# samxuxiang/BrepGen

Measured on NVIDIA H100. Metric: B-reps/sec (1000-step ABC cascade), higher is better.
Workload: dtype f16 x f16 -> f32 (wgmma; split hi+lo weights on in/out-proj; fp32 residual/LN/softmax)

## Files before the change

### brepgen_b200/csrc/attn.cu

```cuda
#include <math.h>

#include "bg_internal.h"
#include "ptx.cuh"


namespace bg {

namespace {

constexpr int DH = 64;
constexpr int NHEAD = 12;
constexpr int DMODEL = 768;
constexpr int BQ = 128;
constexpr int TILE_BYTES = 128 * DH * 2;
constexpr int ST = 2;
constexpr int OFF_Q = 0;
constexpr int OFF_K = TILE_BYTES;
constexpr int OFF_V = OFF_K + ST * TILE_BYTES;
constexpr int OFF_BAR = OFF_V + ST * TILE_BYTES;
constexpr int OFF_MASKW = OFF_BAR + 256;
constexpr int MAX_KB = ATTN_MAX_L / 128;
constexpr int SMEM_BYTES = OFF_MASKW + MAX_KB * 16 + 1024;
constexpr int THREADS = 384;
constexpr int CONSUMER_THREADS = 256;

struct AttnParams {
  __half* out;
  int ldo;
  int B, L, nkb;
  const uint8_t* key_mask;
  const int* blk_list;
  const int* blk_count;
  const uint32_t* blk_words;
  const int* seq_row0;
  const int* seq_len;
  float scale_log2;
};

__device__ __forceinline__ float quad_max(float v) {
  v = fmaxf(v, __shfl_xor_sync(0xffffffffu, v, 1));
  return fmaxf(v, __shfl_xor_sync(0xffffffffu, v, 2));
}
__device__ __forceinline__ float quad_sum(float v) {
  v += __shfl_xor_sync(0xffffffffu, v, 1);
  return v + __shfl_xor_sync(0xffffffffu, v, 2);
}

struct Ring {
  int stage = 0;
  uint32_t phase = 0;
  __device__ __forceinline__ void advance() {
    if (++stage == ST) {
      stage = 0;
      phase ^= 1u;
    }
  }
};

__device__ __forceinline__ void issue_qk(float (&sc)[64], uint32_t q_addr, uint32_t k_addr) {
#pragma unroll
  for (int k = 0; k < DH / 16; ++k)
    wgmma_m64n128k16_ss(sc, make_sw128_desc(q_addr + k * 32), make_sw128_desc(k_addr + k * 32), k > 0 ? 1u : 0u);
  wgmma_commit();
}

__device__ __forceinline__ void issue_pv(float (&o)[DH / 2], const uint32_t (&pa)[8][4], uint32_t v_addr) {
#pragma unroll
  for (int kk = 0; kk < 8; ++kk) wgmma_m64n64k16_rs_bt(o, pa[kk], make_sw128_desc(v_addr + kk * 2048), 1u);
  wgmma_commit();
}

__device__ __forceinline__ void softmax_block(float (&sc)[64], const uint32_t* iw4, float (&m_run)[2], float (&l_run)[2],
                                              float (&alpha)[2], float c, int lane) {
  const uint4 iw = *reinterpret_cast<const uint4*>(iw4);
  if ((iw.x | iw.y | iw.z | iw.w) != 0) {
    const uint32_t inval[4] = {iw.x, iw.y, iw.z, iw.w};
#pragma unroll
    for (int i = 0; i < 16; ++i)
#pragma unroll
      for (int j = 0; j < 2; ++j) {
        const int key = 8 * i + 2 * (lane & 3) + j;
        if ((inval[key >> 5] >> (key & 31)) & 1u) {
          sc[4 * i + j] = -INFINITY;
          sc[4 * i + 2 + j] = -INFINITY;
        }
      }
  }
  float ref[2];
#pragma unroll
  for (int hr = 0; hr < 2; ++hr) {
    float mx = -INFINITY;
#pragma unroll
    for (int i = 0; i < 16; ++i) mx = fmaxf(mx, fmaxf(sc[4 * i + 2 * hr], sc[4 * i + 2 * hr + 1]));
    const float m_new = fmaxf(m_run[hr], quad_max(mx));
    ref[hr] = m_new == -INFINITY ? 0.f : m_new;
    alpha[hr] = ex2((m_run[hr] - ref[hr]) * c);
    m_run[hr] = m_new;
    l_run[hr] *= alpha[hr];
  }
  const float nm0 = -ref[0] * c, nm1 = -ref[1] * c;
#pragma unroll
  for (int i = 0; i < 16; ++i) {
    const float p0 = ex2(fmaf(sc[4 * i], c, nm0)), p1 = ex2(fmaf(sc[4 * i + 1], c, nm0));
    const float p2 = ex2(fmaf(sc[4 * i + 2], c, nm1)), p3 = ex2(fmaf(sc[4 * i + 3], c, nm1));
    l_run[0] += p0 + p1;
    l_run[1] += p2 + p3;
    sc[4 * i] = p0;
    sc[4 * i + 1] = p1;
    sc[4 * i + 2] = p2;
    sc[4 * i + 3] = p3;
  }
}

__device__ __forceinline__ void scale_o(float (&o)[DH / 2], const float (&alpha)[2]) {
#pragma unroll
  for (int i = 0; i < DH / 8; ++i) {
    o[4 * i] *= alpha[0];
    o[4 * i + 1] *= alpha[0];
    o[4 * i + 2] *= alpha[1];
    o[4 * i + 3] *= alpha[1];
  }
}

__device__ __forceinline__ void pack_p(uint32_t (&pa)[8][4], const float (&sc)[64]) {
#pragma unroll
  for (int i = 0; i < 16; ++i) {
    pa[i >> 1][(i & 1) * 2] = pack_half2(sc[4 * i], sc[4 * i + 1]);
    pa[i >> 1][(i & 1) * 2 + 1] = pack_half2(sc[4 * i + 2], sc[4 * i + 3]);
  }
}

__global__ void __launch_bounds__(THREADS, 1)
attn_kernel(const __grid_constant__ CUtensorMap tmQKV, const AttnParams p) {
  extern __shared__ uint8_t smem_raw[];
  uint8_t* smem = reinterpret_cast<uint8_t*>((reinterpret_cast<uintptr_t>(smem_raw) + 1023) & ~uintptr_t(1023));
  uint64_t* bars = reinterpret_cast<uint64_t*>(smem + OFF_BAR);
  uint64_t* q_full = bars;
  uint64_t* k_full = q_full + 1;
  uint64_t* k_empty = k_full + ST;
  uint64_t* v_full = k_empty + ST;
  uint64_t* v_empty = v_full + ST;

  const int warp = threadIdx.x >> 5;
  const int lane = threadIdx.x & 31;
  const int wg = threadIdx.x >> 7;
  const int qgrp = blockIdx.x, h = blockIdx.y, b = blockIdx.z;
  const int row0 = p.seq_row0 ? p.seq_row0[b] : b * p.L;
  const int len = p.seq_len ? p.seq_len[b] : p.L;
  if (qgrp * BQ >= len) return;
  const int nblk = p.blk_count ? p.blk_count[b] : (len + 127) / 128;
  const int* blist = p.blk_list ? p.blk_list + (size_t)b * p.nkb : nullptr;

  if (threadIdx.x == 0) {
    tma_prefetch_desc(&tmQKV);
    mbar_init(q_full, 1);
    for (int i = 0; i < ST; ++i) {
      mbar_init(&k_full[i], 1);
      mbar_init(&k_empty[i], CONSUMER_THREADS);
      mbar_init(&v_full[i], 1);
      mbar_init(&v_empty[i], CONSUMER_THREADS);
    }
    fence_barrier_init();
  }
  uint32_t* maskw = reinterpret_cast<uint32_t*>(smem + OFF_MASKW);
  if (p.blk_words || !p.key_mask) {
    for (int wi = threadIdx.x; wi < nblk * 4; wi += THREADS) {
      uint32_t w;
      if (p.blk_words) {
        w = p.blk_words[((size_t)b * p.nkb + (wi >> 2)) * 4 + (wi & 3)];
      } else {
        const int base = (wi >> 2) * 128 + (wi & 3) * 32;
        w = base + 32 <= len ? 0u : (base >= len ? 0xffffffffu : (0xffffffffu << (len - base)));
      }
      maskw[wi] = w;
    }
  } else {
    for (int wi = warp; wi < nblk * 4; wi += THREADS / 32) {
      const int kb = blist ? blist[wi >> 2] : (wi >> 2);
      const int key = kb * 128 + (wi & 3) * 32 + lane;
      bool bad = key >= len;
      if (!bad) bad = p.key_mask[(size_t)b * p.L + key] != 0;
      const uint32_t w = __ballot_sync(0xffffffffu, bad);
      if (lane == 0) maskw[wi] = w;
    }
  }
  __syncthreads();

  if (wg == 0) {
    setmaxnreg_dec<24>();
    if (warp == 0 && elect_one()) {
      mbar_arrive_expect_tx(q_full, TILE_BYTES);
      tma_load_2d(smem + OFF_Q, &tmQKV, q_full, h * DH, row0 + qgrp * BQ);
      Ring r;
      for (int it = 0; it < nblk; ++it, r.advance()) {
        const int kb = blist ? blist[it] : it;
        const int s = r.stage;
        mbar_wait(&k_empty[s], r.phase ^ 1u);
        mbar_arrive_expect_tx(&k_full[s], TILE_BYTES);
        tma_load_2d(smem + OFF_K + s * TILE_BYTES, &tmQKV, &k_full[s], DMODEL + h * DH, row0 + kb * 128);
        mbar_wait(&v_empty[s], r.phase ^ 1u);
        mbar_arrive_expect_tx(&v_full[s], TILE_BYTES);
        tma_load_2d(smem + OFF_V + s * TILE_BYTES, &tmQKV, &v_full[s], 2 * DMODEL + h * DH, row0 + kb * 128);
      }
    }
    return;
  }

  setmaxnreg_inc<240>();
  const int half = wg - 1;
  const int wq = warp & 3;
  const float c = p.scale_log2;
  const uint32_t q_addr = smem_u32(smem + OFF_Q) + half * 64 * 128;
  float m_run[2] = {-INFINITY, -INFINITY}, l_run[2] = {0.f, 0.f};
  float o[DH / 2];
#pragma unroll
  for (int i = 0; i < DH / 2; ++i) o[i] = 0.f;

  mbar_wait(q_full, 0);
  if (nblk > 0) {
    const uint32_t k_base = smem_u32(smem + OFF_K), v_base = smem_u32(smem + OFF_V);
    Ring kr, vr;
    float sc[64], alpha[2];
    uint32_t pa[8][4];

    mbar_wait(&k_full[kr.stage], kr.phase);
    wgmma_fence();
    issue_qk(sc, q_addr, k_base + kr.stage * TILE_BYTES);
    wgmma_wait<0>();
    wgmma_fence_operand(sc);
    mbar_arrive(&k_empty[kr.stage]);
    kr.advance();
    softmax_block(sc, maskw, m_run, l_run, alpha, c, lane);

#pragma unroll 1
    for (int it = 1; it < nblk; ++it) {
      wgmma_wait<0>();
      wgmma_fence_operand(o);
      if (it >= 2) {
        mbar_arrive(&v_empty[vr.stage]);
        vr.advance();
      }
      scale_o(o, alpha);
      pack_p(pa, sc);
      mbar_wait(&k_full[kr.stage], kr.phase);
      mbar_wait(&v_full[vr.stage], vr.phase);
      wgmma_fence_operand(o);
      wgmma_fence();
      issue_qk(sc, q_addr, k_base + kr.stage * TILE_BYTES);
      issue_pv(o, pa, v_base + vr.stage * TILE_BYTES);
      wgmma_wait<1>();
      wgmma_fence_operand(sc);
      mbar_arrive(&k_empty[kr.stage]);
      kr.advance();
      softmax_block(sc, maskw + it * 4, m_run, l_run, alpha, c, lane);
    }

    wgmma_wait<0>();
    wgmma_fence_operand(o);
    if (nblk >= 2) {
      mbar_arrive(&v_empty[vr.stage]);
      vr.advance();
    }
    scale_o(o, alpha);
    pack_p(pa, sc);
    mbar_wait(&v_full[vr.stage], vr.phase);
    wgmma_fence_operand(o);
    wgmma_fence();
    issue_pv(o, pa, v_base + vr.stage * TILE_BYTES);
    wgmma_wait<0>();
    wgmma_fence_operand(o);
    mbar_arrive(&v_empty[vr.stage]);
  }

#pragma unroll
  for (int hr = 0; hr < 2; ++hr) {
    const float l = quad_sum(l_run[hr]);
    const float inv = l > 0.f ? 1.f / l : 0.f;
    const int row = qgrp * BQ + half * 64 + wq * 16 + hr * 8 + (lane >> 2);
    if (row >= len) continue;
    __half* dst = p.out + ((size_t)row0 + row) * p.ldo + h * DH + 2 * (lane & 3);
#pragma unroll
    for (int i = 0; i < DH / 8; ++i)
      *reinterpret_cast<uint32_t*>(dst + 8 * i) = pack_half2(o[4 * i + 2 * hr] * inv, o[4 * i + 2 * hr + 1] * inv);
  }
}

__global__ void block_list_kernel(const uint8_t* __restrict__ key_mask, int L, int nkb, int* __restrict__ blk_list,
                                  int* __restrict__ blk_count, uint32_t* __restrict__ blk_words) {
  extern __shared__ int sm_bl[];
  int* pos = sm_bl;
  uint32_t* wds = reinterpret_cast<uint32_t*>(sm_bl + nkb);
  const int b = blockIdx.x;
  const int warp = threadIdx.x >> 5, lane = threadIdx.x & 31, nwarp = blockDim.x >> 5;
  for (int kb = warp; kb < nkb; kb += nwarp) {
    bool any = false;
#pragma unroll
    for (int c = 0; c < 4; ++c) {
      const int key = kb * 128 + c * 32 + lane;
      const bool bad = key >= L || key_mask[(size_t)b * L + key] != 0;
      const uint32_t w = __ballot_sync(0xffffffffu, bad);
      any = any || w != 0xffffffffu;
      if (lane == 0) wds[kb * 4 + c] = w;
    }
    if (lane == 0) pos[kb] = any ? 0 : -1;
  }
  __syncthreads();
  if (threadIdx.x == 0) {
    int n = 0;
    for (int kb = 0; kb < nkb; ++kb)
      if (pos[kb] == 0) {
        blk_list[(size_t)b * nkb + n] = kb;
        pos[kb] = n++;
      }
    blk_count[b] = n;
  }
  __syncthreads();
  if (blk_words)
    for (int i = threadIdx.x; i < nkb * 4; i += blockDim.x)
      if (pos[i >> 2] >= 0) blk_words[((size_t)b * nkb + pos[i >> 2]) * 4 + (i & 3)] = wds[i];
}

}

int launch_attention(cudaStream_t st, const AttnArgs& a) {
  BG_REQUIRE(a.qkv && a.out && a.B > 0 && a.L > 0, "attention: bad arguments");
  BG_REQUIRE(a.ldo % 8 == 0, "attention: output pitch must be a multiple of 8");
  BG_REQUIRE(a.L <= ATTN_MAX_L, "attention: sequence longer than 8192 tokens is not supported");
  BG_REQUIRE((a.blk_list == nullptr) == (a.blk_count == nullptr), "attention: blk_list and blk_count go together");
  CUtensorMap tm;
  BG_REQUIRE((a.seq_row0 == nullptr) == (a.seq_len == nullptr), "attention: seq_row0 and seq_len go together");
  BG_REQUIRE(a.seq_len == nullptr || (a.key_mask == nullptr && a.blk_list == nullptr), "attention: variable-length mode takes no mask");
  BG_TRY(make_tmap_2d_f16(&tm, a.qkv, (uint64_t)a.B * (uint64_t)a.L, 3 * DMODEL, 3 * DMODEL, 128));
  AttnParams p;
  p.out = a.out; p.ldo = a.ldo; p.B = a.B; p.L = a.L; p.nkb = (a.L + 127) / 128;
  p.key_mask = a.key_mask; p.blk_list = a.blk_list; p.blk_count = a.blk_count; p.blk_words = a.blk_words;
  p.seq_row0 = a.seq_row0; p.seq_len = a.seq_len;
  p.scale_log2 = 1.4426950408889634f / 8.0f;
  BG_TRY(ensure_dynamic_smem(reinterpret_cast<const void*>(&attn_kernel), SMEM_BYTES));
  dim3 grid((a.L + BQ - 1) / BQ, NHEAD, a.B);
  attn_kernel<<<grid, THREADS, SMEM_BYTES, st>>>(tm, p);
  return check_launch("attn_kernel launch");
}

int launch_build_block_list(cudaStream_t st, const uint8_t* key_mask, int B, int L, int* blk_list, int* blk_count,
                            uint32_t* blk_words) {
  BG_REQUIRE(key_mask && blk_list && blk_count && B > 0 && L > 0, "block list: bad arguments");
  const int nkb = (L + 127) / 128;
  block_list_kernel<<<B, 128, nkb * 5 * sizeof(int), st>>>(key_mask, L, nkb, blk_list, blk_count, blk_words);
  return check_launch("block_list_kernel launch");
}

}
```

### brepgen_b200/csrc/ptx.cuh

```cuda
#pragma once
#include <cuda.h>
#include <cuda_fp16.h>
#include <cuda_runtime.h>
#include <stdint.h>

namespace bg {

__device__ __forceinline__ uint32_t smem_u32(const void* p) { return (uint32_t)__cvta_generic_to_shared(p); }

__device__ __forceinline__ bool elect_one() {
  uint32_t pred;
  asm volatile(
      "{\n\t.reg .pred P;\n\t.reg .b32 R;\n\t"
      "elect.sync R|P, 0xffffffff;\n\t"
      "selp.b32 %0, 1, 0, P;\n\t}\n"
      : "=r"(pred));
  return pred != 0;
}

__device__ __forceinline__ void mbar_init(uint64_t* bar, uint32_t count) {
  asm volatile("mbarrier.init.shared::cta.b64 [%0], %1;" ::"r"(smem_u32(bar)), "r"(count));
}
__device__ __forceinline__ void fence_barrier_init() { asm volatile("fence.mbarrier_init.release.cluster;" ::: "memory"); }
__device__ __forceinline__ void mbar_arrive(uint64_t* bar) {
  asm volatile("mbarrier.arrive.shared::cta.b64 _, [%0];" ::"r"(smem_u32(bar)) : "memory");
}
__device__ __forceinline__ void mbar_arrive_expect_tx(uint64_t* bar, uint32_t bytes) {
  asm volatile("mbarrier.arrive.expect_tx.shared::cta.b64 _, [%0], %1;" ::"r"(smem_u32(bar)), "r"(bytes) : "memory");
}
__device__ __forceinline__ bool mbar_try_wait(uint64_t* bar, uint32_t parity) {
  uint32_t ok;
  asm volatile(
      "{\n\t.reg .pred P;\n\t"
      "mbarrier.try_wait.parity.shared::cta.b64 P, [%1], %2;\n\t"
      "selp.b32 %0, 1, 0, P;\n\t}\n"
      : "=r"(ok)
      : "r"(smem_u32(bar)), "r"(parity)
      : "memory");
  return ok != 0;
}
__device__ __forceinline__ void mbar_wait(uint64_t* bar, uint32_t parity) {
  uint32_t spins = 0;
  while (!mbar_try_wait(bar, parity)) {
    if (++spins > (1u << 26)) asm volatile("trap;");
  }
}

__device__ __forceinline__ void tma_prefetch_desc(const CUtensorMap* m) {
  asm volatile("prefetch.tensormap [%0];" ::"l"(reinterpret_cast<uint64_t>(m)) : "memory");
}
__device__ __forceinline__ void tma_load_2d(void* smem_dst, const CUtensorMap* m, uint64_t* bar, int c0, int c1) {
  asm volatile(
      "cp.async.bulk.tensor.2d.shared::cluster.global.mbarrier::complete_tx::bytes [%0], [%1, {%3, %4}], [%2];"
      ::"r"(smem_u32(smem_dst)), "l"(reinterpret_cast<uint64_t>(m)), "r"(smem_u32(bar)), "r"(c0), "r"(c1)
      : "memory");
}

__device__ __forceinline__ void tma_load_4d(void* smem_dst, const CUtensorMap* m, uint64_t* bar, int c0, int c1, int c2, int c3) {
  asm volatile(
      "cp.async.bulk.tensor.4d.shared::cluster.global.mbarrier::complete_tx::bytes [%0], [%1, {%3, %4, %5, %6}], [%2];"
      ::"r"(smem_u32(smem_dst)), "l"(reinterpret_cast<uint64_t>(m)), "r"(smem_u32(bar)), "r"(c0), "r"(c1), "r"(c2), "r"(c3)
      : "memory");
}

__device__ __forceinline__ void prefetch_l2_bulk(const void* p, uint32_t bytes) {
  asm volatile("cp.async.bulk.prefetch.L2.global [%0], %1;" ::"l"(reinterpret_cast<uint64_t>(p)), "r"(bytes) : "memory");
}

template <uint32_t N>
__device__ __forceinline__ void setmaxnreg_dec() { asm volatile("setmaxnreg.dec.sync.aligned.u32 %0;" ::"n"(N)); }
template <uint32_t N>
__device__ __forceinline__ void setmaxnreg_inc() { asm volatile("setmaxnreg.inc.sync.aligned.u32 %0;" ::"n"(N)); }

__device__ __forceinline__ uint64_t make_sw128_desc(uint32_t smem_addr, uint32_t sbo_bytes = 1024) {
  uint64_t d = 0;
  d |= (uint64_t)((smem_addr & 0x3FFFF) >> 4);
  d |= (uint64_t)1 << 16;
  d |= (uint64_t)((sbo_bytes >> 4) & 0x3FFF) << 32;
  d |= (uint64_t)1 << 62;
  return d;
}

__device__ __forceinline__ void wgmma_fence() { asm volatile("wgmma.fence.sync.aligned;" ::: "memory"); }
__device__ __forceinline__ void wgmma_commit() { asm volatile("wgmma.commit_group.sync.aligned;" ::: "memory"); }
template <int N>
__device__ __forceinline__ void wgmma_wait() { asm volatile("wgmma.wait_group.sync.aligned %0;" ::"n"(N) : "memory"); }
template <int R>
__device__ __forceinline__ void wgmma_fence_operand(float (&d)[R]) {
#pragma unroll
  for (int i = 0; i < R; ++i) asm volatile("" : "+f"(d[i])::"memory");
}

__device__ __forceinline__ void wgmma_m64n256k16_ss(float (&d)[128], uint64_t a_desc, uint64_t b_desc, uint32_t accumulate) {
  asm volatile(
      "{\n\t.reg .pred p;\n\t"
      "setp.ne.b32 p, %130, 0;\n\t"
      "wgmma.mma_async.sync.aligned.m64n256k16.f32.f16.f16 "
      "{%0, %1, %2, %3, %4, %5, %6, %7, %8, %9, %10, %11, %12, %13, %14, %15, "
      "%16, %17, %18, %19, %20, %21, %22, %23, %24, %25, %26, %27, %28, %29, %30, %31, "
      "%32, %33, %34, %35, %36, %37, %38, %39, %40, %41, %42, %43, %44, %45, %46, %47, "
      "%48, %49, %50, %51, %52, %53, %54, %55, %56, %57, %58, %59, %60, %61, %62, %63, "
      "%64, %65, %66, %67, %68, %69, %70, %71, %72, %73, %74, %75, %76, %77, %78, %79, "
      "%80, %81, %82, %83, %84, %85, %86, %87, %88, %89, %90, %91, %92, %93, %94, %95, "
      "%96, %97, %98, %99, %100, %101, %102, %103, %104, %105, %106, %107, %108, %109, %110, %111, "
      "%112, %113, %114, %115, %116, %117, %118, %119, %120, %121, %122, %123, %124, %125, %126, %127}, "
      "%128, %129, p, 1, 1, 0, 0;\n\t}\n"
      : "+f"(d[0]), "+f"(d[1]), "+f"(d[2]), "+f"(d[3]), "+f"(d[4]), "+f"(d[5]), "+f"(d[6]), "+f"(d[7]),
        "+f"(d[8]), "+f"(d[9]), "+f"(d[10]), "+f"(d[11]), "+f"(d[12]), "+f"(d[13]), "+f"(d[14]), "+f"(d[15]),
        "+f"(d[16]), "+f"(d[17]), "+f"(d[18]), "+f"(d[19]), "+f"(d[20]), "+f"(d[21]), "+f"(d[22]), "+f"(d[23]),
        "+f"(d[24]), "+f"(d[25]), "+f"(d[26]), "+f"(d[27]), "+f"(d[28]), "+f"(d[29]), "+f"(d[30]), "+f"(d[31]),
        "+f"(d[32]), "+f"(d[33]), "+f"(d[34]), "+f"(d[35]), "+f"(d[36]), "+f"(d[37]), "+f"(d[38]), "+f"(d[39]),
        "+f"(d[40]), "+f"(d[41]), "+f"(d[42]), "+f"(d[43]), "+f"(d[44]), "+f"(d[45]), "+f"(d[46]), "+f"(d[47]),
        "+f"(d[48]), "+f"(d[49]), "+f"(d[50]), "+f"(d[51]), "+f"(d[52]), "+f"(d[53]), "+f"(d[54]), "+f"(d[55]),
        "+f"(d[56]), "+f"(d[57]), "+f"(d[58]), "+f"(d[59]), "+f"(d[60]), "+f"(d[61]), "+f"(d[62]), "+f"(d[63]),
        "+f"(d[64]), "+f"(d[65]), "+f"(d[66]), "+f"(d[67]), "+f"(d[68]), "+f"(d[69]), "+f"(d[70]), "+f"(d[71]),
        "+f"(d[72]), "+f"(d[73]), "+f"(d[74]), "+f"(d[75]), "+f"(d[76]), "+f"(d[77]), "+f"(d[78]), "+f"(d[79]),
        "+f"(d[80]), "+f"(d[81]), "+f"(d[82]), "+f"(d[83]), "+f"(d[84]), "+f"(d[85]), "+f"(d[86]), "+f"(d[87]),
        "+f"(d[88]), "+f"(d[89]), "+f"(d[90]), "+f"(d[91]), "+f"(d[92]), "+f"(d[93]), "+f"(d[94]), "+f"(d[95]),
        "+f"(d[96]), "+f"(d[97]), "+f"(d[98]), "+f"(d[99]), "+f"(d[100]), "+f"(d[101]), "+f"(d[102]), "+f"(d[103]),
        "+f"(d[104]), "+f"(d[105]), "+f"(d[106]), "+f"(d[107]), "+f"(d[108]), "+f"(d[109]), "+f"(d[110]), "+f"(d[111]),
        "+f"(d[112]), "+f"(d[113]), "+f"(d[114]), "+f"(d[115]), "+f"(d[116]), "+f"(d[117]), "+f"(d[118]), "+f"(d[119]),
        "+f"(d[120]), "+f"(d[121]), "+f"(d[122]), "+f"(d[123]), "+f"(d[124]), "+f"(d[125]), "+f"(d[126]), "+f"(d[127])
      : "l"(a_desc), "l"(b_desc), "r"(accumulate));
}

__device__ __forceinline__ void wgmma_m64n128k16_ss(float (&d)[64], uint64_t a_desc, uint64_t b_desc, uint32_t accumulate) {
  asm volatile(
      "{\n\t.reg .pred p;\n\t"
      "setp.ne.b32 p, %66, 0;\n\t"
      "wgmma.mma_async.sync.aligned.m64n128k16.f32.f16.f16 "
      "{%0, %1, %2, %3, %4, %5, %6, %7, %8, %9, %10, %11, %12, %13, %14, %15, "
      "%16, %17, %18, %19, %20, %21, %22, %23, %24, %25, %26, %27, %28, %29, %30, %31, "
      "%32, %33, %34, %35, %36, %37, %38, %39, %40, %41, %42, %43, %44, %45, %46, %47, "
      "%48, %49, %50, %51, %52, %53, %54, %55, %56, %57, %58, %59, %60, %61, %62, %63}, "
      "%64, %65, p, 1, 1, 0, 0;\n\t}\n"
      : "+f"(d[0]), "+f"(d[1]), "+f"(d[2]), "+f"(d[3]), "+f"(d[4]), "+f"(d[5]), "+f"(d[6]), "+f"(d[7]),
        "+f"(d[8]), "+f"(d[9]), "+f"(d[10]), "+f"(d[11]), "+f"(d[12]), "+f"(d[13]), "+f"(d[14]), "+f"(d[15]),
        "+f"(d[16]), "+f"(d[17]), "+f"(d[18]), "+f"(d[19]), "+f"(d[20]), "+f"(d[21]), "+f"(d[22]), "+f"(d[23]),
        "+f"(d[24]), "+f"(d[25]), "+f"(d[26]), "+f"(d[27]), "+f"(d[28]), "+f"(d[29]), "+f"(d[30]), "+f"(d[31]),
        "+f"(d[32]), "+f"(d[33]), "+f"(d[34]), "+f"(d[35]), "+f"(d[36]), "+f"(d[37]), "+f"(d[38]), "+f"(d[39]),
        "+f"(d[40]), "+f"(d[41]), "+f"(d[42]), "+f"(d[43]), "+f"(d[44]), "+f"(d[45]), "+f"(d[46]), "+f"(d[47]),
        "+f"(d[48]), "+f"(d[49]), "+f"(d[50]), "+f"(d[51]), "+f"(d[52]), "+f"(d[53]), "+f"(d[54]), "+f"(d[55]),
        "+f"(d[56]), "+f"(d[57]), "+f"(d[58]), "+f"(d[59]), "+f"(d[60]), "+f"(d[61]), "+f"(d[62]), "+f"(d[63])
      : "l"(a_desc), "l"(b_desc), "r"(accumulate));
}

__device__ __forceinline__ void wgmma_m64n64k16_rs_bt(float (&d)[32], const uint32_t (&a)[4], uint64_t b_desc, uint32_t accumulate) {
  asm volatile(
      "{\n\t.reg .pred p;\n\t"
      "setp.ne.b32 p, %37, 0;\n\t"
      "wgmma.mma_async.sync.aligned.m64n64k16.f32.f16.f16 "
      "{%0, %1, %2, %3, %4, %5, %6, %7, %8, %9, %10, %11, %12, %13, %14, %15, "
      "%16, %17, %18, %19, %20, %21, %22, %23, %24, %25, %26, %27, %28, %29, %30, %31}, "
      "{%32, %33, %34, %35}, %36, p, 1, 1, 1;\n\t}\n"
      : "+f"(d[0]), "+f"(d[1]), "+f"(d[2]), "+f"(d[3]), "+f"(d[4]), "+f"(d[5]), "+f"(d[6]), "+f"(d[7]),
        "+f"(d[8]), "+f"(d[9]), "+f"(d[10]), "+f"(d[11]), "+f"(d[12]), "+f"(d[13]), "+f"(d[14]), "+f"(d[15]),
        "+f"(d[16]), "+f"(d[17]), "+f"(d[18]), "+f"(d[19]), "+f"(d[20]), "+f"(d[21]), "+f"(d[22]), "+f"(d[23]),
        "+f"(d[24]), "+f"(d[25]), "+f"(d[26]), "+f"(d[27]), "+f"(d[28]), "+f"(d[29]), "+f"(d[30]), "+f"(d[31])
      : "r"(a[0]), "r"(a[1]), "r"(a[2]), "r"(a[3]), "l"(b_desc), "r"(accumulate));
}


__device__ __forceinline__ float ex2(float x) {
  float y;
  asm("ex2.approx.ftz.f32 %0, %1;" : "=f"(y) : "f"(x));
  return y;
}

__device__ __forceinline__ uint32_t pack_half2(float a, float b) {
  __half2 h = __floats2half2_rn(a, b);
  return *reinterpret_cast<uint32_t*>(&h);
}

}
```

Measured before the change: 0.1723.

## Make attention kernel persistent with double-buffered Q/mask and narrow tail blocks

Converts the attention kernel from one CTA per (query tile, head, batch) to a persistent grid sized to the SM count. Each CTA walks work items round-robin, with double-buffered Q tiles and mask words filled by producer warps so the next item's loads overlap the current item's compute. The K/V ring deepens from 2 to 4 stages. The last key block uses narrower wgmma shapes (N=64/32) when its upper keys are fully masked, skipping wasted QK and PV math. This adds barrier and bookkeeping complexity and raises shared-memory use, and the static round-robin assignment may load-balance poorly when sequence lengths vary.

New measurement: 0.1755 (median of 6 runs). 1.8% higher.

```diff
diff --git a/brepgen_b200/csrc/attn.cu b/brepgen_b200/csrc/attn.cu
--- a/brepgen_b200/csrc/attn.cu
+++ b/brepgen_b200/csrc/attn.cu
@@ -13,21 +13,23 @@
 constexpr int DMODEL = 768;
 constexpr int BQ = 128;
 constexpr int TILE_BYTES = 128 * DH * 2;
-constexpr int ST = 2;
+constexpr int ST = 4;
+constexpr int MAX_KB = ATTN_MAX_L / 128;
 constexpr int OFF_Q = 0;
-constexpr int OFF_K = TILE_BYTES;
+constexpr int OFF_K = 2 * TILE_BYTES;
 constexpr int OFF_V = OFF_K + ST * TILE_BYTES;
 constexpr int OFF_BAR = OFF_V + ST * TILE_BYTES;
 constexpr int OFF_MASKW = OFF_BAR + 256;
-constexpr int MAX_KB = ATTN_MAX_L / 128;
-constexpr int SMEM_BYTES = OFF_MASKW + MAX_KB * 16 + 1024;
+constexpr int SMEM_BYTES = OFF_MASKW + 2 * MAX_KB * 16 + 1024;
 constexpr int THREADS = 384;
 constexpr int CONSUMER_THREADS = 256;
+constexpr int WORD_THREADS = 96;
 
 struct AttnParams {
   __half* out;
   int ldo;
   int B, L, nkb;
+  int nqt, nitems;
   const uint8_t* key_mask;
   const int* blk_list;
   const int* blk_count;
@@ -37,6 +39,34 @@
   float scale_log2;
 };
 
+struct Item {
+  int qgrp, h, b, row0, len, nblk;
+};
+
+__device__ __forceinline__ int item_of_round(int i) { return i * gridDim.x + (blockIdx.x + i) % gridDim.x; }
+
+__device__ __forceinline__ bool decode_item(const AttnParams& p, int item, Item& w) {
+  if (item >= p.nitems) return false;
+  w.qgrp = item % p.nqt;
+  const int bh = item / p.nqt;
+  w.h = bh % NHEAD;
+  w.b = bh / NHEAD;
+  w.row0 = p.seq_row0 ? p.seq_row0[w.b] : w.b * p.L;
+  w.len = p.seq_len ? p.seq_len[w.b] : p.L;
+  if (w.qgrp * BQ >= w.len) return false;
+  w.nblk = p.blk_count ? p.blk_count[w.b] : (w.len + 127) / 128;
+  return true;
+}
+
+struct Flip {
+  int buf = 0;
+  uint32_t phase = 0;
+  __device__ __forceinline__ void advance() {
+    buf ^= 1;
+    if (buf == 0) phase ^= 1u;
+  }
+};
+
 __device__ __forceinline__ float quad_max(float v) {
   v = fmaxf(v, __shfl_xor_sync(0xffffffffu, v, 1));
   return fmaxf(v, __shfl_xor_sync(0xffffffffu, v, 2));
@@ -57,26 +87,34 @@
   }
 };
 
+
+template <int NW>
 __device__ __forceinline__ void issue_qk(float (&sc)[64], uint32_t q_addr, uint32_t k_addr) {
 #pragma unroll
-  for (int k = 0; k < DH / 16; ++k)
-    wgmma_m64n128k16_ss(sc, make_sw128_desc(q_addr + k * 32), make_sw128_desc(k_addr + k * 32), k > 0 ? 1u : 0u);
+  for (int k = 0; k < DH / 16; ++k) {
+    const uint64_t qd = make_sw128_desc(q_addr + k * 32), kd = make_sw128_desc(k_addr + k * 32);
+    if constexpr (NW == 128) wgmma_m64n128k16_ss(sc, qd, kd, k > 0 ? 1u : 0u);
+    else if constexpr (NW == 64) wgmma_m64n64k16_ss(reinterpret_cast<float (&)[32]>(sc), qd, kd, k > 0 ? 1u : 0u);
+    else wgmma_m64n32k16_ss(reinterpret_cast<float (&)[16]>(sc), qd, kd, k > 0 ? 1u : 0u);
+  }
   wgmma_commit();
 }
 
+template <int NW>
 __device__ __forceinline__ void issue_pv(float (&o)[DH / 2], const uint32_t (&pa)[8][4], uint32_t v_addr) {
 #pragma unroll
-  for (int kk = 0; kk < 8; ++kk) wgmma_m64n64k16_rs_bt(o, pa[kk], make_sw128_desc(v_addr + kk * 2048), 1u);
+  for (int kk = 0; kk < NW / 16; ++kk) wgmma_m64n64k16_rs_bt(o, pa[kk], make_sw128_desc(v_addr + kk * 2048), 1u);
   wgmma_commit();
 }
 
+template <int NW>
 __device__ __forceinline__ void softmax_block(float (&sc)[64], const uint32_t* iw4, float (&m_run)[2], float (&l_run)[2],
                                               float (&alpha)[2], float c, int lane) {
   const uint4 iw = *reinterpret_cast<const uint4*>(iw4);
   if ((iw.x | iw.y | iw.z | iw.w) != 0) {
     const uint32_t inval[4] = {iw.x, iw.y, iw.z, iw.w};
 #pragma unroll
-    for (int i = 0; i < 16; ++i)
+    for (int i = 0; i < NW / 8; ++i)
 #pragma unroll
       for (int j = 0; j < 2; ++j) {
         const int key = 8 * i + 2 * (lane & 3) + j;
@@ -91,7 +129,7 @@
   for (int hr = 0; hr < 2; ++hr) {
     float mx = -INFINITY;
 #pragma unroll
-    for (int i = 0; i < 16; ++i) mx = fmaxf(mx, fmaxf(sc[4 * i + 2 * hr], sc[4 * i + 2 * hr + 1]));
+    for (int i = 0; i < NW / 8; ++i) mx = fmaxf(mx, fmaxf(sc[4 * i + 2 * hr], sc[4 * i + 2 * hr + 1]));
     const float m_new = fmaxf(m_run[hr], quad_max(mx));
     ref[hr] = m_new == -INFINITY ? 0.f : m_new;
     alpha[hr] = ex2((m_run[hr] - ref[hr]) * c);
@@ -100,7 +138,7 @@
   }
   const float nm0 = -ref[0] * c, nm1 = -ref[1] * c;
 #pragma unroll
-  for (int i = 0; i < 16; ++i) {
+  for (int i = 0; i < NW / 8; ++i) {
     const float p0 = ex2(fmaf(sc[4 * i], c, nm0)), p1 = ex2(fmaf(sc[4 * i + 1], c, nm0));
     const float p2 = ex2(fmaf(sc[4 * i + 2], c, nm1)), p3 = ex2(fmaf(sc[4 * i + 3], c, nm1));
     l_run[0] += p0 + p1;
@@ -122,13 +160,92 @@
   }
 }
 
+template <int NW>
 __device__ __forceinline__ void pack_p(uint32_t (&pa)[8][4], const float (&sc)[64]) {
 #pragma unroll
-  for (int i = 0; i < 16; ++i) {
+  for (int i = 0; i < NW / 8; ++i) {
     pa[i >> 1][(i & 1) * 2] = pack_half2(sc[4 * i], sc[4 * i + 1]);
     pa[i >> 1][(i & 1) * 2 + 1] = pack_half2(sc[4 * i + 2], sc[4 * i + 3]);
   }
 }
+
+struct Consumer {
+  uint64_t *k_full, *k_empty, *v_full, *v_empty;
+  uint32_t k_base, v_base;
+  Ring kr, vr;
+  float c;
+  int lane;
+  float m_run[2], l_run[2], alpha[2];
+  float o[DH / 2];
+  float sc[64];
+  uint32_t pa[8][4];
+
+  template <int NW>
+  __device__ __forceinline__ void first(uint32_t q_addr, const uint32_t* iw4) {
+    mbar_wait(&k_full[kr.stage], kr.phase);
+    wgmma_fence();
+    issue_qk<NW>(sc, q_addr, k_base + kr.stage * TILE_BYTES);
+    wgmma_wait<0>();
+    wgmma_fence_operand(sc);
+    mbar_arrive(&k_empty[kr.stage]);
+    kr.advance();
+    softmax_block<NW>(sc, iw4, m_run, l_run, alpha, c, lane);
+  }
+
+  template <int NW>
+  __device__ __forceinline__ void steady(int it, uint32_t q_addr, const uint32_t* iw4) {
+    wgmma_wait<0>();
+    wgmma_fence_operand(o);
+    if (it >= 2) {
+      mbar_arrive(&v_empty[vr.stage]);
+      vr.advance();
+    }
+    scale_o(o, alpha);
+    pack_p<128>(pa, sc);
+    mbar_wait(&k_full[kr.stage], kr.phase);
+    mbar_wait(&v_full[vr.stage], vr.phase);
+    wgmma_fence_operand(o);
+    wgmma_fence();
+    issue_qk<NW>(sc, q_addr, k_base + kr.stage * TILE_BYTES);
+    issue_pv<128>(o, pa, v_base + vr.stage * TILE_BYTES);
+    wgmma_wait<1>();
+    wgmma_fence_operand(sc);
+    mbar_arrive(&k_empty[kr.stage]);
+    kr.advance();
+    softmax_block<NW>(sc, iw4, m_run, l_run, alpha, c, lane);
+  }
+
+  template <int NW>
+  __device__ __forceinline__ void drain(int nblk) {
+    wgmma_wait<0>();
+    wgmma_fence_operand(o);
+    if (nblk >= 2) {
+      mbar_arrive(&v_empty[vr.stage]);
+      vr.advance();
+    }
+    scale_o(o, alpha);
+    pack_p<NW>(pa, sc);
+    mbar_wait(&v_full[vr.stage], vr.phase);
+    wgmma_fence_operand(o);
+    wgmma_fence();
+    issue_pv<NW>(o, pa, v_base + vr.stage * TILE_BYTES);
+    wgmma_wait<0>();
+    wgmma_fence_operand(o);
+    mbar_arrive(&v_empty[vr.stage]);
+    vr.advance();
+  }
+
+  template <int NW>
+  __device__ __forceinline__ void last(int nblk, uint32_t q_addr, const uint32_t* iw4) {
+    if (nblk > 1) {
+      steady<NW>(nblk - 1, q_addr, iw4);
+      drain<NW>(nblk);
+    } else {
+      first<NW>(q_addr, iw4);
+      drain<NW>(nblk);
+    }
+  }
+};
 
 __global__ void __launch_bounds__(THREADS, 1)
 attn_kernel(const __grid_constant__ CUtensorMap tmQKV, const AttnParams p) {
@@ -136,24 +253,27 @@
   uint8_t* smem = reinterpret_cast<uint8_t*>((reinterpret_cast<uintptr_t>(smem_raw) + 1023) & ~uintptr_t(1023));
   uint64_t* bars = reinterpret_cast<uint64_t*>(smem + OFF_BAR);
   uint64_t* q_full = bars;
-  uint64_t* k_full = q_full + 1;
+  uint64_t* q_empty = q_full + 2;
+  uint64_t* w_full = q_empty + 2;
+  uint64_t* w_empty = w_full + 2;
+  uint64_t* k_full = w_empty + 2;
   uint64_t* k_empty = k_full + ST;
   uint64_t* v_full = k_empty + ST;
   uint64_t* v_empty = v_full + ST;
+  uint32_t* maskw = reinterpret_cast<uint32_t*>(smem + OFF_MASKW);
 
   const int warp = threadIdx.x >> 5;
   const int lane = threadIdx.x & 31;
   const int wg = threadIdx.x >> 7;
-  const int qgrp = blockIdx.x, h = blockIdx.y, b = blockIdx.z;
-  const int row0 = p.seq_row0 ? p.seq_row0[b] : b * p.L;
-  const int len = p.seq_len ? p.seq_len[b] : p.L;
-  if (qgrp * BQ >= len) return;
-  const int nblk = p.blk_count ? p.blk_count[b] : (len + 127) / 128;
-  const int* blist = p.blk_list ? p.blk_list + (size_t)b * p.nkb : nullptr;
 
   if (threadIdx.x == 0) {
     tma_prefetch_desc(&tmQKV);
-    mbar_init(q_full, 1);
+    for (int i = 0; i < 2; ++i) {
+      mbar_init(&q_full[i], 1);
+      mbar_init(&q_empty[i], CONSUMER_THREADS);
+      mbar_init(&w_full[i], WORD_THREADS);
+      mbar_init(&w_empty[i], CONSUMER_THREADS);
+    }
     for (int i = 0; i < ST; ++i) {
       mbar_init(&k_full[i], 1);
       mbar_init(&k_empty[i], CONSUMER_THREADS);
@@ -162,126 +282,120 @@
     }
     fence_barrier_init();
   }
-  uint32_t* maskw = reinterpret_cast<uint32_t*>(smem + OFF_MASKW);
-  if (p.blk_words || !p.key_mask) {
-    for (int wi = threadIdx.x; wi < nblk * 4; wi += THREADS) {
-      uint32_t w;
-      if (p.blk_words) {
-        w = p.blk_words[((size_t)b * p.nkb + (wi >> 2)) * 4 + (wi & 3)];
+  __syncthreads();
+
+  if (wg == 0) {
+    setmaxnreg_dec<32>();
+    if (warp == 0) {
+      if (!elect_one()) return;
+      Flip f;
+      Ring r;
+      for (int i = 0; i * gridDim.x < p.nitems; ++i) {
+        Item w;
+        if (!decode_item(p, item_of_round(i), w)) continue;
+        const int* blist = p.blk_list ? p.blk_list + (size_t)w.b * p.nkb : nullptr;
+        mbar_wait(&q_empty[f.buf], f.phase ^ 1u);
+        mbar_arrive_expect_tx(&q_full[f.buf], TILE_BYTES);
+        tma_load_2d(smem + OFF_Q + f.buf * TILE_BYTES, &tmQKV, &q_full[f.buf], w.h * DH, w.row0 + w.qgrp * BQ);
+        for (int it = 0; it < w.nblk; ++it, r.advance()) {
+          const int kb = blist ? blist[it] : it;
+          const int s = r.stage;
+          mbar_wait(&k_empty[s], r.phase ^ 1u);
+          mbar_arrive_expect_tx(&k_full[s], TILE_BYTES);
+          tma_load_2d(smem + OFF_K + s * TILE_BYTES, &tmQKV, &k_full[s], DMODEL + w.h * DH, w.row0 + kb * 128);
+          mbar_wait(&v_empty[s], r.phase ^ 1u);
+          mbar_arrive_expect_tx(&v_full[s], TILE_BYTES);
+          tma_load_2d(smem + OFF_V + s * TILE_BYTES, &tmQKV, &v_full[s], 2 * DMODEL + w.h * DH, w.row0 + kb * 128);
+        }
+        f.advance();
+      }
+      return;
+    }
+    const int t = threadIdx.x - 32;
+    Flip f;
+    for (int i = 0; i * gridDim.x < p.nitems; ++i) {
+      Item w;
+      if (!decode_item(p, item_of_round(i), w)) continue;
+      uint32_t* mw = maskw + f.buf * (MAX_KB * 4);
+      mbar_wait(&w_empty[f.buf], f.phase ^ 1u);
+      if (p.blk_words || !p.key_mask) {
+        for (int wi = t; wi < w.nblk * 4; wi += WORD_THREADS) {
+          uint32_t wd;
+          if (p.blk_words) {
+            wd = p.blk_words[((size_t)w.b * p.nkb + (wi >> 2)) * 4 + (wi & 3)];
+          } else {
+            const int base = (wi >> 2) * 128 + (wi & 3) * 32;
+            wd = base + 32 <= w.len ? 0u : (base >= w.len ? 0xffffffffu : (0xffffffffu << (w.len - base)));
+          }
+          mw[wi] = wd;
+        }
       } else {
-        const int base = (wi >> 2) * 128 + (wi & 3) * 32;
-        w = base + 32 <= len ? 0u : (base >= len ? 0xffffffffu : (0xffffffffu << (len - base)));
+        const int* blist = p.blk_list ? p.blk_list + (size_t)w.b * p.nkb : nullptr;
+        for (int wi = warp - 1; wi < w.nblk * 4; wi += WORD_THREADS / 32) {
+          const int kb = blist ? blist[wi >> 2] : (wi >> 2);
+          const int key = kb * 128 + (wi & 3) * 32 + lane;
+          bool bad = key >= w.len;
+          if (!bad) bad = p.key_mask[(size_t)w.b * p.L + key] != 0;
+          const uint32_t wd = __ballot_sync(0xffffffffu, bad);
+          if (lane == 0) mw[wi] = wd;
+        }
       }
-      maskw[wi] = w;
-    }
-  } else {
-    for (int wi = warp; wi < nblk * 4; wi += THREADS / 32) {
-      const int kb = blist ? blist[wi >> 2] : (wi >> 2);
-      const int key = kb * 128 + (wi & 3) * 32 + lane;
-      bool bad = key >= len;
-      if (!bad) bad = p.key_mask[(size_t)b * p.L + key] != 0;
-      const uint32_t w = __ballot_sync(0xffffffffu, bad);
-      if (lane == 0) maskw[wi] = w;
-    }
-  }
-  __syncthreads();
-
-  if (wg == 0) {
-    setmaxnreg_dec<24>();
-    if (warp == 0 && elect_one()) {
-      mbar_arrive_expect_tx(q_full, TILE_BYTES);
-      tma_load_2d(smem + OFF_Q, &tmQKV, q_full, h * DH, row0 + qgrp * BQ);
-      Ring r;
-      for (int it = 0; it < nblk; ++it, r.advance()) {
-        const int kb = blist ? blist[it] : it;
-        const int s = r.stage;
-        mbar_wait(&k_empty[s], r.phase ^ 1u);
-        mbar_arrive_expect_tx(&k_full[s], TILE_BYTES);
-        tma_load_2d(smem + OFF_K + s * TILE_BYTES, &tmQKV, &k_full[s], DMODEL + h * DH, row0 + kb * 128);
-        mbar_wait(&v_empty[s], r.phase ^ 1u);
-        mbar_arrive_expect_tx(&v_full[s], TILE_BYTES);
-        tma_load_2d(smem + OFF_V + s * TILE_BYTES, &tmQKV, &v_full[s], 2 * DMODEL + h * DH, row0 + kb * 128);
-      }
+      mbar_arrive(&w_full[f.buf]);
+      f.advance();
     }
     return;
   }
 
-  setmaxnreg_inc<240>();
+  setmaxnreg_inc<232>();
   const int half = wg - 1;
   const int wq = warp & 3;
-  const float c = p.scale_log2;
-  const uint32_t q_addr = smem_u32(smem + OFF_Q) + half * 64 * 128;
-  float m_run[2] = {-INFINITY, -INFINITY}, l_run[2] = {0.f, 0.f};
-  float o[DH / 2];
-#pragma unroll
-  for (int i = 0; i < DH / 2; ++i) o[i] = 0.f;
-
-  mbar_wait(q_full, 0);
-  if (nblk > 0) {
-    const uint32_t k_base = smem_u32(smem + OFF_K), v_base = smem_u32(smem + OFF_V);
-    Ring kr, vr;
-    float sc[64], alpha[2];
-    uint32_t pa[8][4];
-
-    mbar_wait(&k_full[kr.stage], kr.phase);
-    wgmma_fence();
-    issue_qk(sc, q_addr, k_base + kr.stage * TILE_BYTES);
-    wgmma_wait<0>();
-    wgmma_fence_operand(sc);
-    mbar_arrive(&k_empty[kr.stage]);
-    kr.advance();
-    softmax_block(sc, maskw, m_run, l_run, alpha, c, lane);
-
+  Consumer cs;
+  cs.k_full = k_full; cs.k_empty = k_empty; cs.v_full = v_full; cs.v_empty = v_empty;
+  cs.k_base = smem_u32(smem + OFF_K); cs.v_base = smem_u32(smem + OFF_V);
+  cs.c = p.scale_log2;
+  cs.lane = lane;
+  Flip f;
 #pragma unroll 1
-    for (int it = 1; it < nblk; ++it) {
-      wgmma_wait<0>();
-      wgmma_fence_operand(o);
-      if (it >= 2) {
-        mbar_arrive(&v_empty[vr.stage]);
-        vr.advance();
+  for (int i = 0; i * gridDim.x < p.nitems; ++i) {
+    Item w;
+    if (!decode_item(p, item_of_round(i), w)) continue;
+    const uint32_t q_addr = smem_u32(smem + OFF_Q) + f.buf * TILE_BYTES + half * 64 * 128;
+    const uint32_t* mw = maskw + f.buf * (MAX_KB * 4);
+    cs.m_run[0] = cs.m_run[1] = -INFINITY;
+    cs.l_run[0] = cs.l_run[1] = 0.f;
+#pragma unroll
+    for (int i = 0; i < DH / 2; ++i) cs.o[i] = 0.f;
+
+    mbar_wait(&w_full[f.buf], f.phase);
+    mbar_wait(&q_full[f.buf], f.phase);
+    if (w.nblk > 0) {
+      const uint32_t* lw = mw + (w.nblk - 1) * 4;
+      const uint32_t hi = lw[2] & lw[3];
+      const int tailw = hi != 0xffffffffu ? 128 : (lw[1] != 0xffffffffu ? 64 : 32);
+      if (w.nblk > 1) {
+        cs.first<128>(q_addr, mw);
+#pragma unroll 1
+        for (int it = 1; it < w.nblk - 1; ++it) cs.steady<128>(it, q_addr, mw + it * 4);
       }
-      scale_o(o, alpha);
-      pack_p(pa, sc);
-      mbar_wait(&k_full[kr.stage], kr.phase);
-      mbar_wait(&v_full[vr.stage], vr.phase);
-      wgmma_fence_operand(o);
-      wgmma_fence();
-      issue_qk(sc, q_addr, k_base + kr.stage * TILE_BYTES);
-      issue_pv(o, pa, v_base + vr.stage * TILE_BYTES);
-      wgmma_wait<1>();
-      wgmma_fence_operand(sc);
-      mbar_arrive(&k_empty[kr.stage]);
-      kr.advance();
-      softmax_block(sc, maskw + it * 4, m_run, l_run, alpha, c, lane);
-    }
-
-    wgmma_wait<0>();
-    wgmma_fence_operand(o);
-    if (nblk >= 2) {
-      mbar_arrive(&v_empty[vr.stage]);
-      vr.advance();
-    }
-    scale_o(o, alpha);
-    pack_p(pa, sc);
-    mbar_wait(&v_full[vr.stage], vr.phase);
-    wgmma_fence_operand(o);
-    wgmma_fence();
-    issue_pv(o, pa, v_base + vr.stage * TILE_BYTES);
-    wgmma_wait<0>();
-    wgmma_fence_operand(o);
-    mbar_arrive(&v_empty[vr.stage]);
-  }
-
-#pragma unroll
-  for (int hr = 0; hr < 2; ++hr) {
-    const float l = quad_sum(l_run[hr]);
-    const float inv = l > 0.f ? 1.f / l : 0.f;
-    const int row = qgrp * BQ + half * 64 + wq * 16 + hr * 8 + (lane >> 2);
-    if (row >= len) continue;
-    __half* dst = p.out + ((size_t)row0 + row) * p.ldo + h * DH + 2 * (lane & 3);
-#pragma unroll
-    for (int i = 0; i < DH / 8; ++i)
-      *reinterpret_cast<uint32_t*>(dst + 8 * i) = pack_half2(o[4 * i + 2 * hr] * inv, o[4 * i + 2 * hr + 1] * inv);
+      if (tailw == 128) cs.last<128>(w.nblk, q_addr, lw);
+      else if (tailw == 64) cs.last<64>(w.nblk, q_addr, lw);
+      else cs.last<32>(w.nblk, q_addr, lw);
+    }
+    mbar_arrive(&q_empty[f.buf]);
+    mbar_arrive(&w_empty[f.buf]);
+    f.advance();
+
+#pragma unroll
+    for (int hr = 0; hr < 2; ++hr) {
+      const float l = quad_sum(cs.l_run[hr]);
+      const float inv = l > 0.f ? 1.f / l : 0.f;
+      const int row = w.qgrp * BQ + half * 64 + wq * 16 + hr * 8 + (lane >> 2);
+      if (row >= w.len) continue;
+      __half* dst = p.out + ((size_t)w.row0 + row) * p.ldo + w.h * DH + 2 * (lane & 3);
+#pragma unroll
+      for (int i = 0; i < DH / 8; ++i)
+        *reinterpret_cast<uint32_t*>(dst + 8 * i) = pack_half2(cs.o[4 * i + 2 * hr] * inv, cs.o[4 * i + 2 * hr + 1] * inv);
+    }
   }
 }
 
@@ -336,8 +450,10 @@
   p.key_mask = a.key_mask; p.blk_list = a.blk_list; p.blk_count = a.blk_count; p.blk_words = a.blk_words;
   p.seq_row0 = a.seq_row0; p.seq_len = a.seq_len;
   p.scale_log2 = 1.4426950408889634f / 8.0f;
+  p.nqt = (a.L + BQ - 1) / BQ;
+  p.nitems = a.B * NHEAD * p.nqt;
   BG_TRY(ensure_dynamic_smem(reinterpret_cast<const void*>(&attn_kernel), SMEM_BYTES));
-  dim3 grid((a.L + BQ - 1) / BQ, NHEAD, a.B);
+  const int grid = p.nitems < num_sms() ? p.nitems : num_sms();
   attn_kernel<<<grid, THREADS, SMEM_BYTES, st>>>(tm, p);
   return check_launch("attn_kernel launch");
 }
diff --git a/brepgen_b200/csrc/ptx.cuh b/brepgen_b200/csrc/ptx.cuh
--- a/brepgen_b200/csrc/ptx.cuh
+++ b/brepgen_b200/csrc/ptx.cuh
@@ -145,6 +145,33 @@
       : "l"(a_desc), "l"(b_desc), "r"(accumulate));
 }
 
+__device__ __forceinline__ void wgmma_m64n64k16_ss(float (&d)[32], uint64_t a_desc, uint64_t b_desc, uint32_t accumulate) {
+  asm volatile(
+      "{\n\t.reg .pred p;\n\t"
+      "setp.ne.b32 p, %34, 0;\n\t"
+      "wgmma.mma_async.sync.aligned.m64n64k16.f32.f16.f16 "
+      "{%0, %1, %2, %3, %4, %5, %6, %7, %8, %9, %10, %11, %12, %13, %14, %15, "
+      "%16, %17, %18, %19, %20, %21, %22, %23, %24, %25, %26, %27, %28, %29, %30, %31}, "
+      "%32, %33, p, 1, 1, 0, 0;\n\t}\n"
+      : "+f"(d[0]), "+f"(d[1]), "+f"(d[2]), "+f"(d[3]), "+f"(d[4]), "+f"(d[5]), "+f"(d[6]), "+f"(d[7]),
+        "+f"(d[8]), "+f"(d[9]), "+f"(d[10]), "+f"(d[11]), "+f"(d[12]), "+f"(d[13]), "+f"(d[14]), "+f"(d[15]),
+        "+f"(d[16]), "+f"(d[17]), "+f"(d[18]), "+f"(d[19]), "+f"(d[20]), "+f"(d[21]), "+f"(d[22]), "+f"(d[23]),
+        "+f"(d[24]), "+f"(d[25]), "+f"(d[26]), "+f"(d[27]), "+f"(d[28]), "+f"(d[29]), "+f"(d[30]), "+f"(d[31])
+      : "l"(a_desc), "l"(b_desc), "r"(accumulate));
+}
+
+__device__ __forceinline__ void wgmma_m64n32k16_ss(float (&d)[16], uint64_t a_desc, uint64_t b_desc, uint32_t accumulate) {
+  asm volatile(
+      "{\n\t.reg .pred p;\n\t"
+      "setp.ne.b32 p, %18, 0;\n\t"
+      "wgmma.mma_async.sync.aligned.m64n32k16.f32.f16.f16 "
+      "{%0, %1, %2, %3, %4, %5, %6, %7, %8, %9, %10, %11, %12, %13, %14, %15}, "
+      "%16, %17, p, 1, 1, 0, 0;\n\t}\n"
+      : "+f"(d[0]), "+f"(d[1]), "+f"(d[2]), "+f"(d[3]), "+f"(d[4]), "+f"(d[5]), "+f"(d[6]), "+f"(d[7]),
+        "+f"(d[8]), "+f"(d[9]), "+f"(d[10]), "+f"(d[11]), "+f"(d[12]), "+f"(d[13]), "+f"(d[14]), "+f"(d[15])
+      : "l"(a_desc), "l"(b_desc), "r"(accumulate));
+}
+
 __device__ __forceinline__ void wgmma_m64n64k16_rs_bt(float (&d)[32], const uint32_t (&a)[4], uint64_t b_desc, uint32_t accumulate) {
   asm volatile(
       "{\n\t.reg .pred p;\n\t"
```

## Use three consumer warpgroups per attention CTA and deepen KV ring

Applied to the files above, without the earlier changes.

Each attention CTA now handles 192 query rows with three consumer warpgroups instead of 128 rows with two. The K/V ring grows from two to four stages, with a separate Q tensor map for the taller Q tile. The intra-warpgroup software pipeline that overlapped QK of the next block with PV of the current one is replaced by a simple sequential loop, so overlap now comes from running several warpgroups at once. Empty barriers take one arrival per warp, idle warpgroups exit early, and the register budget drops to 160 per thread, which trades per-warpgroup ILP for more K/V reuse and fewer CTAs.

Result: faster. 0.1729 before, 0.1838 after (median of 6 runs) (+6.3%).

```diff
diff --git a/brepgen_b200/csrc/attn.cu b/brepgen_b200/csrc/attn.cu
--- a/brepgen_b200/csrc/attn.cu
+++ b/brepgen_b200/csrc/attn.cu
@@ -11,18 +11,20 @@
 constexpr int DH = 64;
 constexpr int NHEAD = 12;
 constexpr int DMODEL = 768;
-constexpr int BQ = 128;
+constexpr int NCW = 3;
+constexpr int BQ = NCW * 64;
+constexpr int Q_BYTES = BQ * DH * 2;
 constexpr int TILE_BYTES = 128 * DH * 2;
-constexpr int ST = 2;
+constexpr int ST = 4;
 constexpr int OFF_Q = 0;
-constexpr int OFF_K = TILE_BYTES;
+constexpr int OFF_K = Q_BYTES;
 constexpr int OFF_V = OFF_K + ST * TILE_BYTES;
 constexpr int OFF_BAR = OFF_V + ST * TILE_BYTES;
 constexpr int OFF_MASKW = OFF_BAR + 256;
 constexpr int MAX_KB = ATTN_MAX_L / 128;
 constexpr int SMEM_BYTES = OFF_MASKW + MAX_KB * 16 + 1024;
-constexpr int THREADS = 384;
-constexpr int CONSUMER_THREADS = 256;
+constexpr int THREADS = 128 * (NCW + 1);
+static_assert(OFF_K % 1024 == 0, "K / V tiles must start on 1024-byte boundaries (SW128)");
 
 struct AttnParams {
   __half* out;
@@ -131,7 +133,7 @@
 }
 
 __global__ void __launch_bounds__(THREADS, 1)
-attn_kernel(const __grid_constant__ CUtensorMap tmQKV, const AttnParams p) {
+attn_kernel(const __grid_constant__ CUtensorMap tmQ, const __grid_constant__ CUtensorMap tmKV, const AttnParams p) {
   extern __shared__ uint8_t smem_raw[];
   uint8_t* smem = reinterpret_cast<uint8_t*>((reinterpret_cast<uintptr_t>(smem_raw) + 1023) & ~uintptr_t(1023));
   uint64_t* bars = reinterpret_cast<uint64_t*>(smem + OFF_BAR);
@@ -150,15 +152,17 @@
   if (qgrp * BQ >= len) return;
   const int nblk = p.blk_count ? p.blk_count[b] : (len + 127) / 128;
   const int* blist = p.blk_list ? p.blk_list + (size_t)b * p.nkb : nullptr;
+  const int nact = min(NCW, (len - qgrp * BQ + 63) / 64);
 
   if (threadIdx.x == 0) {
-    tma_prefetch_desc(&tmQKV);
+    tma_prefetch_desc(&tmQ);
+    tma_prefetch_desc(&tmKV);
     mbar_init(q_full, 1);
     for (int i = 0; i < ST; ++i) {
       mbar_init(&k_full[i], 1);
-      mbar_init(&k_empty[i], CONSUMER_THREADS);
+      mbar_init(&k_empty[i], nact * 4);
       mbar_init(&v_full[i], 1);
-      mbar_init(&v_empty[i], CONSUMER_THREADS);
+      mbar_init(&v_empty[i], nact * 4);
     }
     fence_barrier_init();
   }
@@ -189,94 +193,64 @@
   if (wg == 0) {
     setmaxnreg_dec<24>();
     if (warp == 0 && elect_one()) {
-      mbar_arrive_expect_tx(q_full, TILE_BYTES);
-      tma_load_2d(smem + OFF_Q, &tmQKV, q_full, h * DH, row0 + qgrp * BQ);
+      mbar_arrive_expect_tx(q_full, Q_BYTES);
+      tma_load_2d(smem + OFF_Q, &tmQ, q_full, h * DH, row0 + qgrp * BQ);
       Ring r;
       for (int it = 0; it < nblk; ++it, r.advance()) {
         const int kb = blist ? blist[it] : it;
         const int s = r.stage;
         mbar_wait(&k_empty[s], r.phase ^ 1u);
         mbar_arrive_expect_tx(&k_full[s], TILE_BYTES);
-        tma_load_2d(smem + OFF_K + s * TILE_BYTES, &tmQKV, &k_full[s], DMODEL + h * DH, row0 + kb * 128);
+        tma_load_2d(smem + OFF_K + s * TILE_BYTES, &tmKV, &k_full[s], DMODEL + h * DH, row0 + kb * 128);
         mbar_wait(&v_empty[s], r.phase ^ 1u);
         mbar_arrive_expect_tx(&v_full[s], TILE_BYTES);
-        tma_load_2d(smem + OFF_V + s * TILE_BYTES, &tmQKV, &v_full[s], 2 * DMODEL + h * DH, row0 + kb * 128);
+        tma_load_2d(smem + OFF_V + s * TILE_BYTES, &tmKV, &v_full[s], 2 * DMODEL + h * DH, row0 + kb * 128);
       }
     }
     return;
   }
 
-  setmaxnreg_inc<240>();
-  const int half = wg - 1;
+  const int cw = wg - 1;
+  if (cw >= nact) return;
+  setmaxnreg_inc<160>();
   const int wq = warp & 3;
   const float c = p.scale_log2;
-  const uint32_t q_addr = smem_u32(smem + OFF_Q) + half * 64 * 128;
+  const uint32_t q_addr = smem_u32(smem + OFF_Q) + cw * 64 * 128;
   float m_run[2] = {-INFINITY, -INFINITY}, l_run[2] = {0.f, 0.f};
   float o[DH / 2];
 #pragma unroll
   for (int i = 0; i < DH / 2; ++i) o[i] = 0.f;
 
   mbar_wait(q_full, 0);
-  if (nblk > 0) {
-    const uint32_t k_base = smem_u32(smem + OFF_K), v_base = smem_u32(smem + OFF_V);
-    Ring kr, vr;
+  const uint32_t k_base = smem_u32(smem + OFF_K), v_base = smem_u32(smem + OFF_V);
+  Ring r;
+#pragma unroll 1
+  for (int it = 0; it < nblk; ++it, r.advance()) {
     float sc[64], alpha[2];
     uint32_t pa[8][4];
-
-    mbar_wait(&k_full[kr.stage], kr.phase);
+    mbar_wait(&k_full[r.stage], r.phase);
     wgmma_fence();
-    issue_qk(sc, q_addr, k_base + kr.stage * TILE_BYTES);
+    issue_qk(sc, q_addr, k_base + r.stage * TILE_BYTES);
     wgmma_wait<0>();
     wgmma_fence_operand(sc);
-    mbar_arrive(&k_empty[kr.stage]);
-    kr.advance();
-    softmax_block(sc, maskw, m_run, l_run, alpha, c, lane);
-
-#pragma unroll 1
-    for (int it = 1; it < nblk; ++it) {
-      wgmma_wait<0>();
-      wgmma_fence_operand(o);
-      if (it >= 2) {
-        mbar_arrive(&v_empty[vr.stage]);
-        vr.advance();
-      }
-      scale_o(o, alpha);
-      pack_p(pa, sc);
-      mbar_wait(&k_full[kr.stage], kr.phase);
-      mbar_wait(&v_full[vr.stage], vr.phase);
-      wgmma_fence_operand(o);
-      wgmma_fence();
-      issue_qk(sc, q_addr, k_base + kr.stage * TILE_BYTES);
-      issue_pv(o, pa, v_base + vr.stage * TILE_BYTES);
-      wgmma_wait<1>();
-      wgmma_fence_operand(sc);
-      mbar_arrive(&k_empty[kr.stage]);
-      kr.advance();
-      softmax_block(sc, maskw + it * 4, m_run, l_run, alpha, c, lane);
-    }
-
+    if (lane == 0) mbar_arrive(&k_empty[r.stage]);
+    softmax_block(sc, maskw + it * 4, m_run, l_run, alpha, c, lane);
+    scale_o(o, alpha);
+    pack_p(pa, sc);
+    mbar_wait(&v_full[r.stage], r.phase);
+    wgmma_fence_operand(o);
+    wgmma_fence();
+    issue_pv(o, pa, v_base + r.stage * TILE_BYTES);
     wgmma_wait<0>();
     wgmma_fence_operand(o);
-    if (nblk >= 2) {
-      mbar_arrive(&v_empty[vr.stage]);
-      vr.advance();
-    }
-    scale_o(o, alpha);
-    pack_p(pa, sc);
-    mbar_wait(&v_full[vr.stage], vr.phase);
-    wgmma_fence_operand(o);
-    wgmma_fence();
-    issue_pv(o, pa, v_base + vr.stage * TILE_BYTES);
-    wgmma_wait<0>();
-    wgmma_fence_operand(o);
-    mbar_arrive(&v_empty[vr.stage]);
+    if (lane == 0) mbar_arrive(&v_empty[r.stage]);
   }
 
 #pragma unroll
   for (int hr = 0; hr < 2; ++hr) {
     const float l = quad_sum(l_run[hr]);
     const float inv = l > 0.f ? 1.f / l : 0.f;
-    const int row = qgrp * BQ + half * 64 + wq * 16 + hr * 8 + (lane >> 2);
+    const int row = qgrp * BQ + cw * 64 + wq * 16 + hr * 8 + (lane >> 2);
     if (row >= len) continue;
     __half* dst = p.out + ((size_t)row0 + row) * p.ldo + h * DH + 2 * (lane & 3);
 #pragma unroll
@@ -327,10 +301,11 @@
   BG_REQUIRE(a.ldo % 8 == 0, "attention: output pitch must be a multiple of 8");
   BG_REQUIRE(a.L <= ATTN_MAX_L, "attention: sequence longer than 8192 tokens is not supported");
   BG_REQUIRE((a.blk_list == nullptr) == (a.blk_count == nullptr), "attention: blk_list and blk_count go together");
-  CUtensorMap tm;
+  CUtensorMap tmQ, tmKV;
   BG_REQUIRE((a.seq_row0 == nullptr) == (a.seq_len == nullptr), "attention: seq_row0 and seq_len go together");
   BG_REQUIRE(a.seq_len == nullptr || (a.key_mask == nullptr && a.blk_list == nullptr), "attention: variable-length mode takes no mask");
-  BG_TRY(make_tmap_2d_f16(&tm, a.qkv, (uint64_t)a.B * (uint64_t)a.L, 3 * DMODEL, 3 * DMODEL, 128));
+  BG_TRY(make_tmap_2d_f16(&tmQ, a.qkv, (uint64_t)a.B * (uint64_t)a.L, 3 * DMODEL, 3 * DMODEL, BQ));
+  BG_TRY(make_tmap_2d_f16(&tmKV, a.qkv, (uint64_t)a.B * (uint64_t)a.L, 3 * DMODEL, 3 * DMODEL, 128));
   AttnParams p;
   p.out = a.out; p.ldo = a.ldo; p.B = a.B; p.L = a.L; p.nkb = (a.L + 127) / 128;
   p.key_mask = a.key_mask; p.blk_list = a.blk_list; p.blk_count = a.blk_count; p.blk_words = a.blk_words;
@@ -338,7 +313,7 @@
   p.scale_log2 = 1.4426950408889634f / 8.0f;
   BG_TRY(ensure_dynamic_smem(reinterpret_cast<const void*>(&attn_kernel), SMEM_BYTES));
   dim3 grid((a.L + BQ - 1) / BQ, NHEAD, a.B);
-  attn_kernel<<<grid, THREADS, SMEM_BYTES, st>>>(tm, p);
+  attn_kernel<<<grid, THREADS, SMEM_BYTES, st>>>(tmQ, tmKV, p);
   return check_launch("attn_kernel launch");
 }
 
```
